# EndMy5uffering/4DGaussianSplatRendering

Hardware: AMD Instinct MI355X
Metric: Gaussians/sec + ms/frame @1080p; sort permutation bit-exact (higher is better)
Workload: dtype f32; 1 GPU; 1,000,000 random 3D splats in a 400^3 cube, single 1080p frame (BASELINE.json configs[1]); splats=1000000, width=1920, height=1080, sort=on, frame_lanes=4, tile_list_entries=1377553, longest_tile_list=477, unordered_draws=3094, staged_list_draws=3094, overflow_reruns=3, depth_sort_passes=3, record_bytes_read_by_projection=64, tiles_composited=14400, tiles=32400, key_index_buffer_pairs=4, lane_streams_rejected_at_create=1

## Files before the change

### 4dgaussiansplatrendering_amd/csrc/gs4d_api.hip

```cpp
#include "gs4d_internal.h"
#include <cstdio>
#include <cstring>
#include <cstdlib>
#include <new>
#include <algorithm>
#include <functional>
#include <vector>
#include <cmath>

using namespace gs4d;

namespace {

constexpr int MAX_LANES = 8;

struct Buffer {
    void* d = nullptr;
    size_t bytes = 0;
    uint64_t version = 0;
    float4* soa = nullptr;
    SoaInfo soa_info;
    size_t soa_n = 0;
    uint64_t soa_version = ~0ull;
    uint64_t soa_builds = 0;
// ... 776 lines not shown
    for (int i = 0; i < 4; ++i) c->u.view[5 * i] = c->u.proj[5 * i] = 1.0f;
    if (const char* ev = getenv("GS4D_LANES")) { const int v = atoi(ev); if (v >= 1 && v <= MAX_LANES) c->nlanes = v; }
    if (const char* ev = getenv("GS4D_FUSE_KEYGEN")) c->defer_order = atoi(ev) != 0;
    if (const char* ev = getenv("GS4D_DRAW_PATH")) { if (!strcmp(ev, "ordered")) c->path_pref = 1; }
    if (const char* ev = getenv("GS4D_RENAME")) c->rename_storage = atoi(ev) != 0;
    if (const char* ev = getenv("GS4D_STAGED_BOX")) c->stage_box_enable = atoi(ev) != 0;
    if (const char* ev = getenv("GS4D_STAGED")) c->stage_enable = atoi(ev) != 0;
    if (const char* ev = getenv("GS4D_SLABS")) { const int v = atoi(ev); if (v >= 1 && v <= (int)V2_MAX_SLABS) { c->slabs = 1; while ((int)c->slabs < v) c->slabs *= 2u; } }
    auto bail = [&](int rc) { g_create_error = c->err; gs4d_destroy(c); return rc; };
    if ((e = create_lane_streams(c)) != hipSuccess) return bail(hipfail(c, e, "hipStreamCreate"));
    for (int i = 0; i < c->nlanes; ++i) {
        Lane& L = c->lanes[i];
        for (hipEvent_t* ev : { &L.ev_emit, &L.ev_tail }) {
            if ((e = hipEventCreateWithFlags(ev, hipEventDisableTiming)) != hipSuccess) return bail(hipfail(c, e, "hipEventCreate"));
            if ((e = hipEventRecord(*ev, L.s)) != hipSuccess) return bail(hipfail(c, e, "hipEventRecord"));
        }
        if ((e = hipHostMalloc((void**)&L.host_total, VERDICT_WORDS * 4, hipHostMallocMapped)) != hipSuccess) return bail(hipfail(c, e, "hipHostMalloc"));
        memset(L.host_total, 0, VERDICT_WORDS * 4);
        if ((e = hipHostGetDevicePointer((void**)&L.host_total_dev, L.host_total, 0)) != hipSuccess) return bail(hipfail(c, e, "hipHostGetDevicePointer"));
        L.depth_sort.err = L.pair_sort.err = L.err_word();
    }
    for (hipEvent_t* ev : { &c->ev_user, &c->ev_readback }) {
        if ((e = hipEventCreateWithFlags(ev, hipEventDisableTiming)) != hipSuccess) return bail(hipfail(c, e, "hipEventCreate"));
    }
    {
        bool ordered = false;
        hipStream_t ls[MAX_LANES];
        for (int i = 0; i < c->nlanes; ++i) ls[i] = c->lanes[i].s;
        if ((e = lds_atomic_order_selftest(ls, c->nlanes, &ordered)) != hipSuccess) return bail(hipfail(c, e, "lds_atomic_order_selftest"));
        c->atomic_rank = ordered;
    }
    const int shape_knob = getenv("GS4D_SORT_SHAPE") ? atoi(getenv("GS4D_SORT_SHAPE")) : 0, rank_knob = getenv("GS4D_SORT_RANK") ? atoi(getenv("GS4D_SORT_RANK")) : 0;
    for (int i = 0; i < c->nlanes; ++i) {
        for (SortScratch* ss : { &c->lanes[i].depth_sort, &c->lanes[i].pair_sort }) { ss->atomic_rank = c->atomic_rank; ss->shape_knob = shape_knob; ss->rank_knob = rank_knob; ss->rb_knob = getenv("GS4D_SORT_RB") ? atoi(getenv("GS4D_SORT_RB")) : 0; }
    }
    int rc = alloc_fbs(c, width, height);
    if (rc) return bail(rc);
    *out = c;
    return GS4D_OK;
}

void gs4d_destroy(gs4d_ctx* c) {
    if (!c) return;
    (void)hipSetDevice(c->device);
    for (int i = 0; i < MAX_LANES; ++i) if (c->lanes[i].s) (void)hipStreamSynchronize(c->lanes[i].s);
    for (auto& b : c->bufs) { if (b.d) (void)hipFree(b.d); if (b.soa) (void)hipFree(b.soa); if (b.bbox_dev) (void)hipFree(b.bbox_dev); if (b.ev_fill) (void)hipEventDestroy(b.ev_fill); if (b.ev_scan) (void)hipEventDestroy(b.ev_scan); }
    for (int i = 0; i < MAX_LANES; ++i) {
        Lane& L = c->lanes[i];
        if (c->fbs[i].mem) (void)hipFree(c->fbs[i].mem);
        if (c->fbs[i].tstate) (void)hipFree(c->fbs[i].tstate);
        if (c->fbs[i].linecnt) (void)hipFree(c->fbs[i].linecnt);
        c->fbs[i].free_planes();
        if (L.line_verts) (void)hipFree(L.line_verts);
        if (L.order_copy) (void)hipFree(L.order_copy);
        if (L.regen_keys) (void)hipFree(L.regen_keys);
        if (L.compact_counts) (void)hipFree(L.compact_counts);
        if (L.spatial_scratch) (void)hipFree(L.spatial_scratch);
        if (L.cut_scratch) (void)hipFree(L.cut_scratch);
        for (auto& sp : L.spare) { if (sp.d) (void)hipFree(sp.d); for (hipEvent_t e : sp.ev) if (e) (void)hipEventDestroy(e); }
        if (L.proj) (void)hipFree(L.proj);
        if (L.trects) (void)hipFree(L.trects);
        if (L.pair_keys) (void)hipFree(L.pair_keys);
        tile_lists_free(L.tl);
        sort_scratch_free(L.depth_sort); sort_scratch_free(L.pair_sort); bin_scratch_free(L.bin);
        if (L.host_total) (void)hipHostFree(L.host_total);
        if (L.ev_emit) (void)hipEventDestroy(L.ev_emit);
        if (L.ev_tail) (void)hipEventDestroy(L.ev_tail);
// ... 920 lines not shown
```

### 4dgaussiansplatrendering_amd/csrc/gs4d_internal.h

```cpp
#pragma once
#include <hip/hip_runtime.h>
#include <stdint.h>
#include <stddef.h>
#include <string>
#include <vector>
#include "../../include/gs4d.h"

namespace gs4d {

constexpr int TILE = 8;
constexpr int PROJ_FLOATS = 16;


enum class Outputs : int { Colour = 0, Aux = 1, Ids = 2 };
constexpr bool has_aux(Outputs o) { return o >= Outputs::Aux; }
constexpr bool has_ids(Outputs o) { return o >= Outputs::Ids; }
static_assert(sizeof(gs4d_record_stat) == 16 && offsetof(gs4d_record_stat, wsum) == 8, "the 64-bit sum is naturally aligned in a 16-byte record");
struct StatOut { gs4d_record_stat* rec = nullptr; uint32_t n = 0; };
struct Target {
    float4* fb; uint32_t* tstate; uint32_t epoch; float4 clear;
    Outputs out; float2* aux; uint32_t* ids;
    const float* z = nullptr;
    StatOut stats;
};

struct Uniforms {
    float view[16];
    float proj[16];
    float time;
    float min_opacity;
};

constexpr int VERDICT_WORDS = 16;
enum TotalWord : int { TOT_ENTRIES = 0, TOT_FLAGS = 1, TOT_COUNT_LO = 2, TOT_COUNT_HI = 3, TOT_LONGEST_LIST = 4, TOT_UNUSED_5 = 5, TOT_UNUSED_6 = 6, TOT_SCAN_ARRIVALS = 7, TOT_TICKET = 8, TOT_ABORT = 9 };
enum HostWord : int { HT_ENTRIES = 0, HT_FLAGS = 1, HT_COUNT_LO = 2, HT_COUNT_HI = 3, HT_ERROR = 4, HT_LONGEST_LIST = 5, HT_LONGEST_RUN = 6, HT_FULLEST_BUCKET = 7, HT_FULLEST_SEG = 8, HT_USED_BOX = 9 };
static_assert(TOT_ABORT < VERDICT_WORDS && HT_USED_BOX < VERDICT_WORDS, "the highest word of either layout fits the arrays");
constexpr uint32_t VF_CAPACITY = 1u, VF_LIST = 2u, VF_STAGED_MISS = 4u;

struct SortScratch {
    uint32_t* keys2 = nullptr; uint32_t* vals2 = nullptr; size_t cap = 0;
    uint32_t* hist = nullptr; size_t hist_cap = 0;
    int flip = 0;
    bool hist_pending = false;
    int acc_flip = 0;
    int hist_bits = 32;
    int hist_rb = 8;
    int rb_knob = 0;
    uint32_t hist_bias = 0;
    uint32_t epoch = 0;
    bool atomic_rank = false;
    int shape_knob = 0, rank_knob = 0;
    uint32_t* totals = nullptr;
    uint32_t* err = nullptr;
    struct Resident { const void* fn = nullptr; uint32_t groups = 0; } resident[16];
};
hipError_t sort_scratch_reserve(hipStream_t st, SortScratch& s, size_t n);
void sort_scratch_free(SortScratch& s);
hipError_t radix_sort_pairs(hipStream_t st, SortScratch& s, uint32_t* keys, uint32_t* vals, size_t n, const uint32_t* n_dev, int key_bits, bool have_hist, bool identity_vals = false);
uint32_t* sort_hist_slot(hipStream_t st, SortScratch& s, size_t n_hint, hipError_t* e_out);
int sort_plan_rb(const SortScratch& s, size_t n, int key_bits);
int sort_plan_passes(int key_bits, int rb);
hipError_t lds_atomic_order_selftest(const hipStream_t* streams, int nstreams, bool* ordered);
enum { SOA_FULL = 0, SOA_SYM = 1, SOA_STATIC3D = 2 };
struct SoaInfo { int layout = SOA_FULL; float consts[8] = { 0 }; };
struct KeySrc;
hipError_t launch_keygen(hipStream_t st, const float4* pos, const float4* sig3, const SoaInfo& info, size_t n, const KeySrc& ks, float* keys, uint32_t* idx, uint32_t* ghist, int rb, uint32_t span, uint32_t* err);

template <class T> inline hipError_t grow_device_array(hipStream_t st, T*& p, size_t& cap, size_t want, size_t elem_bytes = sizeof(T)) {
    if (cap >= want) return hipSuccess;
    hipError_t e = hipStreamSynchronize(st); if (e != hipSuccess) return e;
    if (p) (void)hipFree(p);
    p = nullptr; cap = 0;
    if ((e = hipMalloc(&p, want * elem_bytes)) != hipSuccess) { p = nullptr; return e; }
    cap = want;
    return hipSuccess;
}

constexpr int OS_MAX_PASSES = 4;
constexpr int OS_REPL = 8;
constexpr uint32_t OS_MAX_BINS = 512;
constexpr size_t OS_SLOT_WORDS = (size_t)OS_REPL * OS_MAX_PASSES * OS_MAX_BINS;
#ifdef __HIPCC__
__device__ __forceinline__ void os_hist_clear(uint32_t (*h)[OS_MAX_BINS], uint32_t tid) {
#pragma unroll
// ... 208 lines not shown
```

### 4dgaussiansplatrendering_amd/csrc/sort.hip

```cpp
#include "gs4d_internal.h"
#include <algorithm>
#include <cstdlib>
#include <cstdio>
#include <vector>

namespace gs4d {

__global__ __launch_bounds__(256) void k_keygen(const float4* __restrict__ pos, const float4* __restrict__ sig3, uint32_t n, float t,
                                                float camx, float camy, float camz, float4 vrow2 , int key_mode,
                                                float* __restrict__ keys, uint32_t* __restrict__ idx, uint32_t* __restrict__ ghist , int rb ,
                                                uint32_t bias , uint32_t span , uint32_t* __restrict__ err,
                                                float4 csig3, float cmut ) {
    __shared__ uint32_t h[OS_MAX_PASSES][OS_MAX_BINS];
    os_hist_clear(h, threadIdx.x);
    __syncthreads();
    for (uint32_t i0 = blockIdx.x * 256u; i0 < n; i0 += gridDim.x * 256u) {
        const uint32_t i = i0 + threadIdx.x;
        const bool in = i < n;
        float key = 0.0f;
        if (in) {
            float4 p = pos[i];
            float4 s = csig3;
            if (sig3) s = sig3[i]; else p.w = cmut;
            if (key_mode == GS4D_KEY_REF_INV_EUCLID) {
                float ct = t - p.w;
                float x = p.x + s.x * ct;
                float y = p.y + s.y * ct;
                float z = p.z + s.z * ct;
                float dx = x - camx, dy = y - camy, dz = z - camz;
                key = 1.0f / sqrtf(dx * dx + dy * dy + dz * dz);
            } else {
                float k = (1.0f / s.w) * (t - p.w);
                float x = p.x + k * s.x, y = p.y + k * s.y, z = p.z + k * s.z;
                float zv = ((vrow2.x * x + vrow2.y * y) + vrow2.z * z) + vrow2.w;
                key = 1.0f / fmaxf(-zv, 1e-20f);
            }
// ... 30 lines not shown
struct OsBufs { uint32_t* k[3]; uint32_t* v[3]; };

__device__ __forceinline__ uint32_t wave_incl_scan_u32(uint32_t v, uint32_t lane) {
#pragma unroll
    for (int off = 1; off < 64; off <<= 1) { const uint32_t t = __shfl_up(v, off, 64); if (lane >= (unsigned)off) v += t; }
    return v;
}
__global__ __launch_bounds__(256) void k_os_hist(const uint32_t* __restrict__ keys, uint32_t n_cap, const uint32_t* __restrict__ n_dev, int passes, int rb,
                                                 uint32_t* __restrict__ ghist ) {
    __shared__ uint32_t h[OS_MAX_PASSES][OS_MAX_BINS];
    const uint32_t n = n_dev ? min(*n_dev, n_cap) : n_cap;
    const uint32_t tid = threadIdx.x;
    os_hist_clear(h, tid);
    __syncthreads();
    const uint32_t nvec = n / 4u;
    const uint4* k4 = reinterpret_cast<const uint4*>(keys);
    const uint32_t stride = gridDim.x * 256u;
    for (uint32_t i0 = blockIdx.x * 256u + tid; i0 < nvec; i0 += 4u * stride) {
        uint4 kk[4];
        bool in[4];
#pragma unroll
        for (int u = 0; u < 4; ++u) { const uint32_t i = i0 + u * stride; in[u] = i < nvec; kk[u] = in[u] ? k4[i] : make_uint4(0, 0, 0, 0); }
#pragma unroll
        for (int u = 0; u < 4; ++u) {
            os_hist_add(h, kk[u].x, in[u], passes, rb); os_hist_add(h, kk[u].y, in[u], passes, rb);
            os_hist_add(h, kk[u].z, in[u], passes, rb); os_hist_add(h, kk[u].w, in[u], passes, rb);
        }
    }
    if (blockIdx.x == 0) { const bool in = tid < (n & 3u); os_hist_add(h, in ? keys[nvec * 4u + tid] : 0u, in, passes, rb); }
    __syncthreads();
    os_hist_flush(h, ghist, passes, tid);
}

__device__ __forceinline__ bool os_schedule(uint32_t live, int passes, int p, int& src, int& dst, int& executed, int& total) {
    const uint32_t all = (1u << passes) - 1u;
    live &= all;
    int k = __popc(live);
    if (k == 1) { const uint32_t deadm = all & ~live; live |= deadm & (0u - deadm); ++k; }
    total = k;
    const int j = __popc(live & ((1u << p) - 1u));
    executed = j;
    if (!((live >> p) & 1u)) return false;
    auto buf_at = [k](int i) { if (k & 1) { if (i <= 2) return i; return (i - 3) & 1; } return i & 1; };
    src = buf_at(j);
    dst = buf_at(j + 1);
    return true;
}

__device__ __forceinline__ uint32_t os_tword(uint32_t epoch, uint32_t count) { return ((epoch & 0x3FFFFu) << 14) | count; }
__device__ __forceinline__ bool os_tpublished(uint32_t w, uint32_t epoch) { return (w >> 14) == (epoch & 0x3FFFFu); }


template <int LB, int BINS>
__device__ __forceinline__ uint32_t os_tiles_finish(const uint32_t* st, int32_t hi, int rows, int k0, uint32_t sum, uint32_t tid, uint32_t epoch, uint32_t* err) {
    uint32_t spins = 0;
    while (true) {
        while (true) {
            __builtin_amdgcn_s_sleep(8);
            const uint32_t w = __hip_atomic_load(st + (size_t)(hi - k0) * (uint32_t)BINS + tid, __ATOMIC_RELAXED, __HIP_MEMORY_SCOPE_AGENT);
            if (os_tpublished(w, epoch)) { sum += w & 0x3FFFu; break; }
            if (++spins > (1u << 20)) { __hip_atomic_store(err, 1u, __ATOMIC_RELAXED, __HIP_MEMORY_SCOPE_SYSTEM); return sum; }
        }
        if (++k0 >= rows) return sum;
        uint32_t sv[LB];
#pragma unroll
        for (int k = 0; k < LB; ++k) sv[k] = (k >= k0 && k < rows) ? __hip_atomic_load(st + (size_t)(hi - k) * (uint32_t)BINS + tid, __ATOMIC_RELAXED, __HIP_MEMORY_SCOPE_AGENT) : 0u;
        bool missing = false;
#pragma unroll
        for (int k = 0; k < LB; ++k) {
            if (missing || k < k0 || k >= rows) continue;
            if (!os_tpublished(sv[k], epoch)) { k0 = k; missing = true; continue; }
            sum += sv[k] & 0x3FFFu;
        }
        if (!missing) return sum;
    }
}

template <int LB, int BINS>
__device__ __forceinline__ uint32_t os_acc_finish(const uint32_t* acc, uint32_t t, int rows, int k0, uint32_t sum, uint32_t expect, uint32_t tid, uint32_t* err) {
// ... 48 lines not shown
    const uint32_t* sacc = acc + (size_t)acc_groups * (uint32_t)BINS;
    for (uint32_t t = 0; t < sup; t += 16u) {
        const int rows = (int)min(16u, sup - t);
        uint32_t sv[16];
#pragma unroll
        for (int k = 0; k < 16; ++k) sv[k] = k < rows ? __hip_atomic_load(sacc + (size_t)(t + k) * (uint32_t)BINS + tid, __ATOMIC_RELAXED, __HIP_MEMORY_SCOPE_AGENT) : 0u;
        int miss = -1;
#pragma unroll
        for (int k = 0; k < 16; ++k) {
            if (miss >= 0 || k >= rows) continue;
            if ((sv[k] >> 24) != OS_SUPER) { miss = k; continue; }
            sum_s += sv[k] & 0xFFFFFFu;
        }
        if (miss >= 0) sum_s = os_acc_finish<16, BINS>(sacc, t, rows, miss, sum_s, OS_SUPER, tid, err);
    }
    if (miss_t >= 0) sum_t = os_tiles_finish<(int)OS_GROUP, BINS>(st, hi, rows_t, miss_t, sum_t, tid, epoch, err);
    if (miss_g >= 0) sum_g = os_acc_finish<(int)OS_SUPER, BINS>(acc, g0, rows_g, miss_g, sum_g, OS_GROUP, tid, err);
    return sum_t + sum_g + sum_s;
}

template <int THREADS, int BINS>
__device__ __forceinline__ uint32_t digit_excl_scan(uint32_t v, uint32_t* tmp , uint32_t tid) {
    const uint32_t lane = tid & 63u, w = tid >> 6;
    const uint32_t inc = wave_incl_scan_u32(tid < (uint32_t)BINS ? v : 0u, lane);
    __syncthreads();
    if (lane == 63u && w < (uint32_t)(BINS / 64)) tmp[w] = inc;
    __syncthreads();
    uint32_t base = 0;
#pragma unroll
    for (int k = 0; k < BINS / 64 - 1; ++k) if ((unsigned)k < w) base += tmp[k];
    return base + inc - v;
}

template <int THREADS, int ITEMS, bool ATOMIC_RANK, int RB>
__global__ __launch_bounds__(THREADS) void k_os_pass(OsBufs bufs, uint32_t n_cap, const uint32_t* __restrict__ n_dev, int pass, int passes,
                                                     const uint32_t* __restrict__ ghist , uint32_t* __restrict__ ghist_other ,
                                                     uint32_t* status , uint32_t* acc , uint32_t* acc_next , uint32_t acc_groups, uint32_t acc_words,
                                                     uint32_t epoch, uint32_t* err,
                                                     uint32_t* ticket , uint32_t* ticket_next , uint32_t bias, int identity_vals ,
                                                     u64* stamps ) {
    constexpr uint32_t TILE_KEYS = THREADS * ITEMS;
    constexpr int WAVES = THREADS / 64;
    constexpr uint32_t BINS = 1u << RB;
    static_assert(BINS <= (uint32_t)THREADS && BINS <= OS_MAX_BINS && BINS >= 64u, "one thread per digit");
    static_assert(TILE_KEYS < (1u << 14), "tile-level look-back words carry 14-bit counts");
    static_assert((uint64_t)TILE_KEYS * OS_GROUP * OS_SUPER < (1u << 24) && OS_GROUP < 256u && OS_SUPER < 256u, "accumulators are {arrivals:8, sum:24}");
    __shared__ uint32_t skeys[TILE_KEYS];
    __shared__ uint32_t svals[TILE_KEYS];
    __shared__ uint32_t wcnt[WAVES][BINS];
    __shared__ uint32_t loff[BINS];
    __shared__ uint32_t gpos[BINS];
    __shared__ uint32_t s_tmp[BINS / 64];
    __shared__ uint32_t s_dead;
    __shared__ uint32_t s_tile;

    const uint32_t n = n_dev ? min(*n_dev, n_cap) : n_cap;
    const uint32_t tid = threadIdx.x, lane = tid & 63u, w = tid >> 6;
    if (tid == 0) s_tile = atomicAdd(ticket, 1u);
    if (tid == 1u) s_dead = 0u;
    if (tid == 2u && blockIdx.x == 0) __hip_atomic_store(ticket_next, 0u, __ATOMIC_RELAXED, __HIP_MEMORY_SCOPE_AGENT);
    for (uint32_t q = tid; q < WAVES * BINS; q += THREADS) (&wcnt[0][0])[q] = 0u;
    uint32_t tot = 0, dead = 0;
    if (tid < BINS) {
        for (int q = 0; q < passes; ++q) {
            uint32_t g = 0;
#pragma unroll
            for (int r = 0; r < OS_REPL; ++r) g += ghist[(r * OS_MAX_PASSES + q) * OS_MAX_BINS + tid];
            if (q == pass) tot = g;
            if (g == n) dead |= 1u << q;
        }
    }
    __syncthreads();
    if (dead) atomicOr(&s_dead, dead);
    const uint32_t ntiles = (n + TILE_KEYS - 1u) / TILE_KEYS;
    for (uint32_t q = blockIdx.x * THREADS + tid; q < acc_words; q += gridDim.x * THREADS) acc_next[q] = 0u;
    if (pass == 0 && blockIdx.x == 0) { for (uint32_t q = tid; q < OS_SLOT_WORDS; q += THREADS) ghist_other[q] = 0u; }
    __syncthreads();
    uint32_t tile = s_tile;
    if (tile >= ntiles) return;
    const int shift = RB * pass;
    int src, dst, executed, total;
    if (!os_schedule(~s_dead, passes, pass, src, dst, executed, total)) {
        if (identity_vals && pass == 0 && total == 0) { for (uint32_t i = blockIdx.x * THREADS + tid; i < n; i += gridDim.x * THREADS) bufs.v[0][i] = i; }
        return;
    }
    const bool make_identity = identity_vals && executed == 0;
    const uint32_t* __restrict__ keys_in = bufs.k[src]; const uint32_t* __restrict__ vals_in = bufs.v[src];
    uint32_t* __restrict__ keys_out = bufs.k[dst]; uint32_t* __restrict__ vals_out = bufs.v[dst];
    uint32_t digit_base = 0;
    bool first = true;
    const uint32_t ngroups = (ntiles + OS_GROUP - 1u) / OS_GROUP, nsuper = (ngroups + OS_SUPER - 1u) / OS_SUPER;

    while (true) {
        OS_STAMP(0);
        const uint32_t tbase = tile * TILE_KEYS;
        const uint32_t wbase = tbase + w * (64u * ITEMS);
        uint32_t key[ITEMS], val[ITEMS], rank[ITEMS];
#pragma unroll
        for (int j = 0; j < ITEMS; ++j) {
            const uint32_t i = wbase + j * 64u + lane;
            const bool valid = i < n;
            key[j] = valid ? keys_in[i] : 0xFFFFFFFFu;
            val[j] = !valid ? 0u : make_identity ? i : vals_in[i];
        }
        if (first) { digit_base = digit_excl_scan<THREADS, (int)BINS>(tot, s_tmp, tid); first = false; }
        OS_STAMP(1);

        if (ATOMIC_RANK) {
#pragma unroll
            for (int j = 0; j < ITEMS; ++j) {
                const bool valid = (wbase + j * 64u + lane) < n;
                const uint32_t d = ((key[j] - bias) >> shift) & (BINS - 1u);
                rank[j] = valid ? atomicAdd(&wcnt[w][d], 1u) : 0u;
            }
        } else {
            const uint64_t lt = (1ull << lane) - 1ull;
            volatile uint32_t* wc = wcnt[w];
#pragma unroll
            for (int j = 0; j < ITEMS; ++j) {
                const bool valid = (wbase + j * 64u + lane) < n;
                const uint32_t d = ((key[j] - bias) >> shift) & (BINS - 1u);
                uint64_t m = __ballot(valid);
#pragma unroll
                for (int b = 0; b < RB; ++b) {
                    const bool bit = (d >> b) & 1u;
                    const uint64_t bal = __ballot(bit);
                    m &= bit ? bal : ~bal;
                }
                rank[j] = 0;
                if (valid) {
                    const uint32_t c = wc[d];
                    rank[j] = c + (uint32_t)__popcll(m & lt);
                    __builtin_amdgcn_wave_barrier();
                    if ((m & lt) == 0) wc[d] = c + (uint32_t)__popcll(m);
                }
                __builtin_amdgcn_wave_barrier();
            }
        }
        __syncthreads();
        uint32_t cnt = 0;
        uint32_t garr = 0;
        const uint32_t grp = tile / OS_GROUP, sup = grp / OS_SUPER;
        if (tid < BINS) {
#pragma unroll
            for (int k = 0; k < WAVES; ++k) { const uint32_t t = wcnt[k][tid]; wcnt[k][tid] = cnt; cnt += t; }
            __hip_atomic_store(status + (size_t)tile * BINS + tid, os_tword(epoch, cnt), __ATOMIC_RELAXED, __HIP_MEMORY_SCOPE_AGENT);
            if (sup + 1u < nsuper) garr = __hip_atomic_fetch_add(acc + (size_t)grp * BINS + tid, (1u << 24) | cnt, __ATOMIC_RELAXED, __HIP_MEMORY_SCOPE_AGENT);
            else if (grp + 1u < ngroups) (void)__hip_atomic_fetch_add(acc + (size_t)grp * BINS + tid, (1u << 24) | cnt, __ATOMIC_RELAXED, __HIP_MEMORY_SCOPE_AGENT);
        }
        OS_STAMP(2);
        const uint32_t lo_ = digit_excl_scan<THREADS, (int)BINS>(cnt, s_tmp, tid);
        if (tid < BINS) loff[tid] = lo_;
        __syncthreads();
#pragma unroll
        for (int j = 0; j < ITEMS; ++j) {
            if ((wbase + j * 64u + lane) < n) {
                const uint32_t d = ((key[j] - bias) >> shift) & (BINS - 1u);
                const uint32_t l = loff[d] + wcnt[w][d] + rank[j];
                skeys[l] = key[j];
                svals[l] = val[j];
            }
        }
        OS_STAMP(3);
        if (tid < BINS) {
            if (sup + 1u < nsuper && (garr >> 24) == OS_GROUP - 1u)
                (void)__hip_atomic_fetch_add(acc + (size_t)(acc_groups + sup) * BINS + tid, (1u << 24) | ((garr & 0xFFFFFFu) + cnt), __ATOMIC_RELAXED, __HIP_MEMORY_SCOPE_AGENT);
            const uint32_t prefix = os_lookback<(int)BINS>(status, acc, acc_groups, tile, tid, epoch, err);
            gpos[tid] = digit_base + prefix;
        }
        __syncthreads();
        OS_STAMP(4);
        const uint32_t tcount = min(TILE_KEYS, n - tbase);
#pragma unroll
        for (int j = 0; j < ITEMS; ++j) {
            const uint32_t l = j * THREADS + tid;
            if (l < tcount) {
                const uint32_t k = skeys[l];
                const uint32_t d = ((k - bias) >> shift) & (BINS - 1u);
                const uint32_t o = gpos[d] + (l - loff[d]);
                if (o >= n) { __hip_atomic_store(err, 3u, __ATOMIC_RELAXED, __HIP_MEMORY_SCOPE_SYSTEM); continue; }
                if (ITEMS >= 12) { keys_out[o] = k; vals_out[o] = svals[l]; }
                else { __builtin_nontemporal_store(k, keys_out + o); __builtin_nontemporal_store(svals[l], vals_out + o); }
            }
        }
        OS_STAMP(5);
        if (gridDim.x >= ntiles) return;
        uint32_t next = 0;
        if (tid == 0) next = atomicAdd(ticket, 1u);
        __syncthreads();
        if (tid == 0) s_tile = next;
        for (uint32_t q = tid; q < WAVES * BINS; q += THREADS) (&wcnt[0][0])[q] = 0u;
        __syncthreads();
        tile = s_tile;
        if (tile >= ntiles) return;
    }
}

__global__ __launch_bounds__(256) void k_lds_order_test(uint32_t* __restrict__ bad) {
    __shared__ uint32_t cnt[4][256];
    const uint32_t tid = threadIdx.x, lane = tid & 63u, w = tid >> 6;
    uint32_t errors = 0;
    for (uint32_t round = 0; round < 96u; ++round) {
#pragma unroll
        for (int k = 0; k < 4; ++k) cnt[k][tid] = 0u;
        __syncthreads();
        const uint32_t bins = round % 6u == 0u ? 1u : round % 6u == 1u ? 2u : round % 6u == 2u ? 3u : round % 6u == 3u ? 7u : round % 6u == 4u ? 64u : 256u;
        uint32_t x = (blockIdx.x * 256u + tid) * 2654435761u + round * 40503u; x ^= x >> 15; x *= 2246822519u; x ^= x >> 13;
        const uint32_t d = x % bins;
        const bool active = ((x >> 20) & 7u) != 0u;
        uint64_t m = __ballot(active);
#pragma unroll
        for (int b = 0; b < 8; ++b) { const bool bit = (d >> b) & 1u; const uint64_t bal = __ballot(bit); m &= bit ? bal : ~bal; }
        if (active) {
            const uint32_t got = atomicAdd(&cnt[w][d], 1u);
            const uint32_t want = (uint32_t)__popcll(m & ((1ull << lane) - 1ull));
            if (got != want) ++errors;
            const uint32_t got2 = atomicAdd(&cnt[w][d], 1u);
            if (got2 != (uint32_t)__popcll(m) + want) ++errors;
        }
        __syncthreads();
    }
    if (errors) atomicAdd(bad, errors);
}

hipError_t lds_atomic_order_selftest(const hipStream_t* streams, int nstreams, bool* ordered) {
    *ordered = false;
    if (nstreams < 1) return hipErrorInvalidValue;
    if (nstreams > 8) nstreams = 8;
    uint32_t* d = nullptr; uint32_t h[8] = { 1, 1, 1, 1, 1, 1, 1, 1 };
    hipError_t e = hipMalloc(&d, 4 * (size_t)nstreams);
    if (e != hipSuccess) return e;
    for (int i = 0; i < nstreams && e == hipSuccess; ++i) e = hipMemsetAsync(d + i, 0, 4, streams[i]);
    for (int i = 0; i < nstreams && e == hipSuccess; ++i) { k_lds_order_test<<<dim3(512), dim3(256), 0, streams[i]>>>(d + i); e = hipGetLastError(); }
    for (int i = 0; i < nstreams && e == hipSuccess; ++i) e = hipMemcpyAsync(&h[i], d + i, 4, hipMemcpyDeviceToHost, streams[i]);
    for (int i = 0; i < nstreams; ++i) { const hipError_t e2 = hipStreamSynchronize(streams[i]); if (e == hipSuccess) e = e2; }
    (void)hipFree(d);
    bool ok = e == hipSuccess;
    for (int i = 0; i < nstreams; ++i) ok = ok && h[i] == 0;
    *ordered = ok;
    return e;
}

hipError_t sort_scratch_reserve(hipStream_t st, SortScratch& s, size_t n) {
    hipError_t e;
    if (s.cap < n) {
        e = grow_device_array(st, s.keys2, s.cap, n, 16);
        s.vals2 = s.keys2 ? s.keys2 + 2 * s.cap : nullptr;
        if (e != hipSuccess) return e;
    }
    const size_t tiles = (s.cap + 1023) / 1024;
    const size_t groups = tiles / OS_GROUP + 2, supers = groups / OS_SUPER + 2;
    const size_t words = 2 * OS_SLOT_WORDS + (tiles + 2 + 2 * 2 * (groups + supers)) * OS_MAX_BINS;
    if (s.hist_cap < words) {
        uint32_t* nh = nullptr;
        if ((e = hipMalloc(&nh, words * 4)) != hipSuccess) return e;
        if ((e = hipMemsetAsync(nh, 0, words * 4, st)) != hipSuccess) return e;
        if (s.hist) {
            if ((e = hipMemcpyAsync(nh, s.hist, 2 * OS_SLOT_WORDS * 4, hipMemcpyDeviceToDevice, st)) != hipSuccess) return e;
            (void)hipStreamSynchronize(st); (void)hipFree(s.hist);
        }
        s.hist = nh; s.hist_cap = words;
    }
    if (!s.totals) {
        if (const char* e0 = getenv("GS4D_TEST_EPOCH0")) s.epoch = (uint32_t)strtoul(e0, nullptr, 0);
    }
    if (!s.totals) { if ((e = hipMalloc(&s.totals, 256 * 4)) != hipSuccess) return e; if ((e = hipMemsetAsync(s.totals, 0, 1024, st)) != hipSuccess) return e; }
    return hipSuccess;
}

void sort_scratch_free(SortScratch& s) {
    if (s.keys2) (void)hipFree(s.keys2);
    if (s.hist) (void)hipFree(s.hist);
    if (s.totals) (void)hipFree(s.totals);
    s = SortScratch();
}

uint32_t* sort_hist_slot(hipStream_t st, SortScratch& s, size_t n_hint, hipError_t* e_out) {
    hipError_t e = sort_scratch_reserve(st, s, n_hint);
    if (e == hipSuccess && s.hist_pending) e = hipMemsetAsync(s.hist + (s.flip ? OS_SLOT_WORDS : 0), 0, OS_SLOT_WORDS * 4, st);
    if (e_out) *e_out = e;
    if (e != hipSuccess) return nullptr;
    s.hist_pending = true;
    return s.hist + (s.flip ? OS_SLOT_WORDS : 0);
}

template <int THREADS, int ITEMS, bool ATOMIC_RANK, int RB>
static hipError_t onesweep(hipStream_t st, SortScratch& s, uint32_t* keys, uint32_t* vals, size_t n, const uint32_t* n_dev, int passes, bool have_hist, bool identity_vals) {
    const uint32_t tile_keys = THREADS * ITEMS;
    const uint32_t tiles = (uint32_t)((n + tile_keys - 1) / tile_keys);
    uint32_t resident = 0;
    {
        const void* const fn = reinterpret_cast<const void*>(&k_os_pass<THREADS, ITEMS, ATOMIC_RANK, RB>);
        SortScratch::Resident* slot = nullptr;
        for (auto& r : s.resident) { if (r.fn == fn) { resident = r.groups; break; } if (!r.fn && !slot) slot = &r; }
        if (!resident) {
            int per_cu = 0, dev = 0, cus = 0;
            if (hipOccupancyMaxActiveBlocksPerMultiprocessor(&per_cu, k_os_pass<THREADS, ITEMS, ATOMIC_RANK, RB>, THREADS, 0) != hipSuccess || per_cu < 1) per_cu = 1;
            if (hipGetDevice(&dev) != hipSuccess || hipDeviceGetAttribute(&cus, hipDeviceAttributeMultiprocessorCount, dev) != hipSuccess || cus < 1) cus = 256;
            resident = (uint32_t)per_cu * (uint32_t)cus;
            if (slot) { slot->fn = fn; slot->groups = resident; }
        }
    }
    const uint32_t grid = std::min(tiles, resident);
    uint32_t* ghist = s.hist + (s.flip ? OS_SLOT_WORDS : 0);
    uint32_t* ghist_other = s.hist + (s.flip ? 0 : OS_SLOT_WORDS);
    hipError_t e;
    const uint32_t bias = have_hist ? s.hist_bias : 0u;
    s.hist_bias = 0;
    if (!have_hist) {
        if (s.hist_pending) { if ((e = hipMemsetAsync(ghist, 0, OS_SLOT_WORDS * 4, st)) != hipSuccess) return e; }
        const uint32_t hist_blocks = (uint32_t)std::min<size_t>((n / 16 + 255) / 256 + 1, 256);
        k_os_hist<<<dim3(hist_blocks), dim3(256), 0, st>>>(keys, (uint32_t)n, n_dev, passes, RB, ghist);
    }
    s.hist_pending = false;
    s.flip ^= 1;
#ifdef GS4D_TUNING
    static const char* stampf = getenv("GS4D_SORT_STAMP_FILE");
    static const int stamp_pass = getenv("GS4D_SORT_STAMP_PASS") ? atoi(getenv("GS4D_SORT_STAMP_PASS")) : 0;
#else
    const char* stampf = nullptr; const int stamp_pass = 0;
#endif
    u64* stamps = nullptr;
    if (stampf && hipMalloc(&stamps, (size_t)tiles * 64) != hipSuccess) stamps = nullptr;
    uint32_t* status = s.hist + 2 * OS_SLOT_WORDS;
    const size_t cap_tiles = (s.cap + 1023) / 1024, cap_groups = cap_tiles / OS_GROUP + 2, cap_supers = cap_groups / OS_SUPER + 2;
    const size_t acc_words = (cap_groups + cap_supers) * OS_MAX_BINS;
    uint32_t* acc_base = status + (cap_tiles + 2) * OS_MAX_BINS;
    OsBufs b;
    b.k[0] = keys; b.v[0] = vals;
    b.k[1] = s.keys2; b.v[1] = s.vals2;
    b.k[2] = s.keys2 + s.cap; b.v[2] = s.vals2 + s.cap;
    for (int p = 0; p < passes; ++p) {
        ++s.epoch;
        if ((s.epoch & 0x3FFFFu) == 0u) {
            if ((e = hipMemsetAsync(status, 0, (s.hist_cap - 2 * OS_SLOT_WORDS) * 4, st)) != hipSuccess) return e;
            ++s.epoch;
        }
        k_os_pass<THREADS, ITEMS, ATOMIC_RANK, RB><<<dim3(grid), dim3(THREADS), 0, st>>>(b, (uint32_t)n, n_dev, p, passes, ghist, ghist_other, status, acc_base + (s.acc_flip ? acc_words : 0), acc_base + (s.acc_flip ? 0 : acc_words), (uint32_t)cap_groups, (uint32_t)acc_words,
                                                                         s.epoch & 0x3FFFFFFFu,
                                                                         s.err ? s.err : s.totals, s.totals + 64 + (s.acc_flip ? 1 : 0), s.totals + 64 + (s.acc_flip ? 0 : 1), bias, identity_vals ? 1 : 0, (stampf && p == stamp_pass) ? stamps : nullptr);
        s.acc_flip ^= 1;
    }
    if (stampf && stamps) {
        (void)hipStreamSynchronize(st);
        std::vector<u64> hs((size_t)tiles * 8);
        (void)hipMemcpy(hs.data(), stamps, hs.size() * 8, hipMemcpyDeviceToHost);
        FILE* f = fopen(stampf, "w");
        if (f) { for (uint32_t t = 0; t < tiles; ++t) { for (int k = 0; k < 6; ++k) fprintf(f, "%llu ", hs[t * 8 + k] - hs[0]); fprintf(f, "\n"); } fclose(f); }
        (void)hipFree(stamps);
    }
    return hipGetLastError();
}

int sort_plan_rb(const SortScratch& s, size_t n, int key_bits) {
    (void)n;
    if (s.rb_knob == 8 || s.rb_knob == 9) return (s.rb_knob == 9 && (s.shape_knob == 1 || s.shape_knob == 4)) ? 8 : s.rb_knob;
    if (s.shape_knob == 1 || s.shape_knob == 4) return 8;
    const int p8 = std::max(2, (key_bits + 7) / 8), p9 = std::max(2, (key_bits + 8) / 9);
    return p9 < p8 ? 9 : 8;
}
int sort_plan_passes(int key_bits, int rb) { return std::min(OS_MAX_PASSES, std::max(2, (key_bits + rb - 1) / rb)); }

hipError_t radix_sort_pairs(hipStream_t st, SortScratch& s, uint32_t* keys, uint32_t* vals, size_t n, const uint32_t* n_dev, int key_bits, bool have_hist, bool identity_vals) {
    if (n <= 1) { if (n == 1 && identity_vals) return hipMemsetAsync(vals, 0, 4, st); return hipSuccess; }
    if (n >= (1ull << 32) - 1) return hipErrorInvalidValue;
    hipError_t e = sort_scratch_reserve(st, s, n);
    if (e != hipSuccess) return e;
    const int rb = have_hist ? s.hist_rb : sort_plan_rb(s, n, key_bits);
    if (rb != 8 && rb != 9) return hipErrorInvalidValue;
    const int passes = sort_plan_passes(key_bits, rb);
    int shape = s.shape_knob ? s.shape_knob : 5;
    (void)n;
    if (rb == 9 && shape == 5 && !s.shape_knob) shape = 6;
// ... 18 lines not shown
```

Before: 10.61 billion splats/s.

## Add opt-in single-launch onesweep radix sort with cross-pass done counters

Adds a variant of the onesweep pass kernel that runs all digit passes in one launch. Work items are ordered pass-major and blocks spin on per-pass done counters before starting the next pass, replacing separate kernel launches with in-kernel dependency waits and a second alternating accumulator buffer. It is gated behind GS4D_SORT_ONE_LAUNCH and defaults off. The change also adds a grid-size knob and a min-waves launch bound for 512-thread configurations, which can change register allocation on the default path.

```diff
diff --git a/4dgaussiansplatrendering_amd/csrc/gs4d_api.hip b/4dgaussiansplatrendering_amd/csrc/gs4d_api.hip
--- a/4dgaussiansplatrendering_amd/csrc/gs4d_api.hip
+++ b/4dgaussiansplatrendering_amd/csrc/gs4d_api.hip
@@ -832,7 +832,8 @@
     }
     const int shape_knob = getenv("GS4D_SORT_SHAPE") ? atoi(getenv("GS4D_SORT_SHAPE")) : 0, rank_knob = getenv("GS4D_SORT_RANK") ? atoi(getenv("GS4D_SORT_RANK")) : 0;
     for (int i = 0; i < c->nlanes; ++i) {
-        for (SortScratch* ss : { &c->lanes[i].depth_sort, &c->lanes[i].pair_sort }) { ss->atomic_rank = c->atomic_rank; ss->shape_knob = shape_knob; ss->rank_knob = rank_knob; ss->rb_knob = getenv("GS4D_SORT_RB") ? atoi(getenv("GS4D_SORT_RB")) : 0; }
+        for (SortScratch* ss : { &c->lanes[i].depth_sort, &c->lanes[i].pair_sort }) { ss->atomic_rank = c->atomic_rank; ss->shape_knob = shape_knob; ss->rank_knob = rank_knob; ss->rb_knob = getenv("GS4D_SORT_RB") ? atoi(getenv("GS4D_SORT_RB")) : 0;
+                                                                                   ss->one_launch_knob = getenv("GS4D_SORT_ONE_LAUNCH") ? (atoi(getenv("GS4D_SORT_ONE_LAUNCH")) != 0) : -1; ss->grid_knob = getenv("GS4D_SORT_GRID") ? atoi(getenv("GS4D_SORT_GRID")) : 0; }
     }
     int rc = alloc_fbs(c, width, height);
     if (rc) return bail(rc);
diff --git a/4dgaussiansplatrendering_amd/csrc/gs4d_internal.h b/4dgaussiansplatrendering_amd/csrc/gs4d_internal.h
--- a/4dgaussiansplatrendering_amd/csrc/gs4d_internal.h
+++ b/4dgaussiansplatrendering_amd/csrc/gs4d_internal.h
@@ -50,6 +50,9 @@
     uint32_t epoch = 0;
     bool atomic_rank = false;
     int shape_knob = 0, rank_knob = 0;
+    int one_launch_knob = -1;
+    int grid_knob = 0;
+    int done_flip = 0;
     uint32_t* totals = nullptr;
     uint32_t* err = nullptr;
     struct Resident { const void* fn = nullptr; uint32_t groups = 0; } resident[16];
diff --git a/4dgaussiansplatrendering_amd/csrc/sort.hip b/4dgaussiansplatrendering_amd/csrc/sort.hip
--- a/4dgaussiansplatrendering_amd/csrc/sort.hip
+++ b/4dgaussiansplatrendering_amd/csrc/sort.hip
@@ -2,6 +2,7 @@
 #include <algorithm>
 #include <cstdlib>
 #include <cstdio>
+#include <type_traits>
 #include <vector>
 
 namespace gs4d {
@@ -98,11 +99,15 @@
     os_hist_flush(h, ghist, passes, tid);
 }
 
-__device__ __forceinline__ bool os_schedule(uint32_t live, int passes, int p, int& src, int& dst, int& executed, int& total) {
+__device__ __forceinline__ uint32_t os_executed_mask(uint32_t live, int passes) {
     const uint32_t all = (1u << passes) - 1u;
     live &= all;
-    int k = __popc(live);
-    if (k == 1) { const uint32_t deadm = all & ~live; live |= deadm & (0u - deadm); ++k; }
+    if (__popc(live) == 1) { const uint32_t deadm = all & ~live; live |= deadm & (0u - deadm); }
+    return live;
+}
+__device__ __forceinline__ bool os_schedule(uint32_t live, int passes, int p, int& src, int& dst, int& executed, int& total) {
+    live = os_executed_mask(live, passes);
+    const int k = __popc(live);
     total = k;
     const int j = __popc(live & ((1u << p) - 1u));
     executed = j;
@@ -111,6 +116,10 @@
     src = buf_at(j);
     dst = buf_at(j + 1);
     return true;
+}
+__device__ __forceinline__ int os_nth_executed(uint32_t executed_mask, int j) {
+    for (int k = 0; k < j; ++k) executed_mask &= executed_mask - 1u;
+    return __ffs((int)executed_mask) - 1;
 }
 
 __device__ __forceinline__ uint32_t os_tword(uint32_t epoch, uint32_t count) { return ((epoch & 0x3FFFFu) << 14) | count; }
@@ -225,16 +234,19 @@
     return base + inc - v;
 }
 
-template <int THREADS, int ITEMS, bool ATOMIC_RANK, int RB>
-__global__ __launch_bounds__(THREADS) void k_os_pass(OsBufs bufs, uint32_t n_cap, const uint32_t* __restrict__ n_dev, int pass, int passes,
+#define OS_MIN_WAVES(T, I, R) (((T) == 512 && !((I) == 16 && (R) == 9)) ? 4 : 1)
+template <int THREADS, int ITEMS, bool ATOMIC_RANK, int RB, bool ONE>
+__global__ __launch_bounds__(THREADS, OS_MIN_WAVES(THREADS, ITEMS, RB)) void k_os_pass(OsBufs bufs, uint32_t n_cap, const uint32_t* __restrict__ n_dev, int pass , int passes,
                                                      const uint32_t* __restrict__ ghist , uint32_t* __restrict__ ghist_other ,
                                                      uint32_t* status , uint32_t* acc , uint32_t* acc_next , uint32_t acc_groups, uint32_t acc_words,
                                                      uint32_t epoch, uint32_t* err,
                                                      uint32_t* ticket , uint32_t* ticket_next , uint32_t bias, int identity_vals ,
-                                                     u64* stamps ) {
+                                                     u64* stamps ,
+                                                     uint32_t* acc_mid , uint32_t* done , uint32_t* done_next ) {
     constexpr uint32_t TILE_KEYS = THREADS * ITEMS;
     constexpr int WAVES = THREADS / 64;
     constexpr uint32_t BINS = 1u << RB;
+    constexpr uint32_t OS_ABANDON = 0xFFFFFFFFu;
     static_assert(BINS <= (uint32_t)THREADS && BINS <= OS_MAX_BINS && BINS >= 64u, "one thread per digit");
     static_assert(TILE_KEYS < (1u << 14), "tile-level look-back words carry 14-bit counts");
     static_assert((uint64_t)TILE_KEYS * OS_GROUP * OS_SUPER < (1u << 24) && OS_GROUP < 256u && OS_SUPER < 256u, "accumulators are {arrivals:8, sum:24}");
@@ -252,37 +264,93 @@
     if (tid == 0) s_tile = atomicAdd(ticket, 1u);
     if (tid == 1u) s_dead = 0u;
     if (tid == 2u && blockIdx.x == 0) __hip_atomic_store(ticket_next, 0u, __ATOMIC_RELAXED, __HIP_MEMORY_SCOPE_AGENT);
+    if (ONE && tid >= 64u && tid < 64u + (uint32_t)OS_MAX_PASSES && blockIdx.x == 0) __hip_atomic_store(done_next + (tid - 64u), 0u, __ATOMIC_RELAXED, __HIP_MEMORY_SCOPE_AGENT);
     for (uint32_t q = tid; q < WAVES * BINS; q += THREADS) (&wcnt[0][0])[q] = 0u;
     uint32_t tot = 0, dead = 0;
+    uint32_t totq[OS_MAX_PASSES] = { 0u, 0u, 0u, 0u };
+    static_assert(OS_MAX_PASSES == 4, "totq");
     if (tid < BINS) {
-        for (int q = 0; q < passes; ++q) {
-            uint32_t g = 0;
-#pragma unroll
-            for (int r = 0; r < OS_REPL; ++r) g += ghist[(r * OS_MAX_PASSES + q) * OS_MAX_BINS + tid];
-            if (q == pass) tot = g;
-            if (g == n) dead |= 1u << q;
+        if (ONE) {
+#pragma unroll
+            for (int q = 0; q < OS_MAX_PASSES; ++q) {
+                if (q >= passes) continue;
+                uint32_t g = 0;
+#pragma unroll
+                for (int r = 0; r < OS_REPL; ++r) g += ghist[(r * OS_MAX_PASSES + q) * OS_MAX_BINS + tid];
+                totq[q] = g;
+                if (g == n) dead |= 1u << q;
+            }
+        } else {
+            for (int q = 0; q < passes; ++q) {
+                uint32_t g = 0;
+#pragma unroll
+                for (int r = 0; r < OS_REPL; ++r) g += ghist[(r * OS_MAX_PASSES + q) * OS_MAX_BINS + tid];
+                if (q == pass) tot = g;
+                if (g == n) dead |= 1u << q;
+            }
         }
     }
     __syncthreads();
     if (dead) atomicOr(&s_dead, dead);
     const uint32_t ntiles = (n + TILE_KEYS - 1u) / TILE_KEYS;
     for (uint32_t q = blockIdx.x * THREADS + tid; q < acc_words; q += gridDim.x * THREADS) acc_next[q] = 0u;
-    if (pass == 0 && blockIdx.x == 0) { for (uint32_t q = tid; q < OS_SLOT_WORDS; q += THREADS) ghist_other[q] = 0u; }
+    if ((ONE || pass == 0) && blockIdx.x == 0) { for (uint32_t q = tid; q < OS_SLOT_WORDS; q += THREADS) ghist_other[q] = 0u; }
     __syncthreads();
     uint32_t tile = s_tile;
-    if (tile >= ntiles) return;
-    const int shift = RB * pass;
-    int src, dst, executed, total;
-    if (!os_schedule(~s_dead, passes, pass, src, dst, executed, total)) {
-        if (identity_vals && pass == 0 && total == 0) { for (uint32_t i = blockIdx.x * THREADS + tid; i < n; i += gridDim.x * THREADS) bufs.v[0][i] = i; }
-        return;
-    }
-    const bool make_identity = identity_vals && executed == 0;
-    const uint32_t* __restrict__ keys_in = bufs.k[src]; const uint32_t* __restrict__ vals_in = bufs.v[src];
-    uint32_t* __restrict__ keys_out = bufs.k[dst]; uint32_t* __restrict__ vals_out = bufs.v[dst];
+    uint32_t item = tile, nitems = ntiles;
+    int shift = RB * pass;
+    int src = 0, dst = 0, executed = 0, total = 0;
+    int cur_j = 0;
+    uint32_t ep = epoch;
+    uint32_t* acc_cur = acc;
+    bool first = true;
+    if (ONE) {
+        const uint32_t xm = os_executed_mask(~s_dead, passes);
+        total = __popc(xm);
+        if (total == 0) {
+            if (identity_vals) { for (uint32_t i = blockIdx.x * THREADS + tid; i < n; i += gridDim.x * THREADS) bufs.v[0][i] = i; }
+            return;
+        }
+        nitems = ntiles * (uint32_t)total;
+        if (item >= nitems) return;
+        cur_j = (int)(item / ntiles);
+        tile = item - (uint32_t)cur_j * ntiles;
+        if (cur_j > 0) {
+            if (tid == 0) {
+                uint32_t spins = 0;
+                while (__hip_atomic_load(done + (cur_j - 1), __ATOMIC_RELAXED, __HIP_MEMORY_SCOPE_AGENT) < ntiles) {
+                    __builtin_amdgcn_s_sleep(8);
+                    if (++spins > (1u << 20)) { __hip_atomic_store(err, 1u, __ATOMIC_RELAXED, __HIP_MEMORY_SCOPE_SYSTEM); s_tile = OS_ABANDON; break; }
+                }
+                __builtin_amdgcn_fence(__ATOMIC_ACQUIRE, "agent");
+                asm volatile("s_waitcnt vmcnt(0)" ::: "memory");
+            }
+            __syncthreads();
+            if (s_tile == OS_ABANDON) return;
+        }
+        const int p = os_nth_executed(xm, cur_j);
+        (void)os_schedule(~s_dead, passes, p, src, dst, executed, total);
+        shift = RB * p;
+        tot = p == 0 ? totq[0] : p == 1 ? totq[1] : p == 2 ? totq[2] : totq[3];
+        ep = epoch + (uint32_t)cur_j;
+        acc_cur = (cur_j & 1) ? acc_mid : acc;
+    } else {
+        if (tile >= ntiles) return;
+        if (!os_schedule(~s_dead, passes, pass, src, dst, executed, total)) {
+            if (identity_vals && pass == 0 && total == 0) { for (uint32_t i = blockIdx.x * THREADS + tid; i < n; i += gridDim.x * THREADS) bufs.v[0][i] = i; }
+            return;
+        }
+    }
+    bool make_identity = identity_vals && executed == 0;
+    using In = std::conditional_t<ONE, const uint32_t*, const uint32_t* __restrict__>;
+    using Out = std::conditional_t<ONE, uint32_t*, uint32_t* __restrict__>;
+    In keys_in = bufs.k[src]; In vals_in = bufs.v[src];
+    Out keys_out = bufs.k[dst]; Out vals_out = bufs.v[dst];
     uint32_t digit_base = 0;
-    bool first = true;
     const uint32_t ngroups = (ntiles + OS_GROUP - 1u) / OS_GROUP, nsuper = (ngroups + OS_SUPER - 1u) / OS_SUPER;
+#ifdef GS4D_TUNING
+    if (ONE && stamps && shift != RB * pass) stamps = nullptr;
+#endif
 
     while (true) {
         OS_STAMP(0);
@@ -337,9 +405,15 @@
         if (tid < BINS) {
 #pragma unroll
             for (int k = 0; k < WAVES; ++k) { const uint32_t t = wcnt[k][tid]; wcnt[k][tid] = cnt; cnt += t; }
-            __hip_atomic_store(status + (size_t)tile * BINS + tid, os_tword(epoch, cnt), __ATOMIC_RELAXED, __HIP_MEMORY_SCOPE_AGENT);
-            if (sup + 1u < nsuper) garr = __hip_atomic_fetch_add(acc + (size_t)grp * BINS + tid, (1u << 24) | cnt, __ATOMIC_RELAXED, __HIP_MEMORY_SCOPE_AGENT);
-            else if (grp + 1u < ngroups) (void)__hip_atomic_fetch_add(acc + (size_t)grp * BINS + tid, (1u << 24) | cnt, __ATOMIC_RELAXED, __HIP_MEMORY_SCOPE_AGENT);
+            __hip_atomic_store(status + (size_t)tile * BINS + tid, os_tword(ep, cnt), __ATOMIC_RELAXED, __HIP_MEMORY_SCOPE_AGENT);
+            if (sup + 1u < nsuper) garr = __hip_atomic_fetch_add(acc_cur + (size_t)grp * BINS + tid, (1u << 24) | cnt, __ATOMIC_RELAXED, __HIP_MEMORY_SCOPE_AGENT);
+            else if (grp + 1u < ngroups) (void)__hip_atomic_fetch_add(acc_cur + (size_t)grp * BINS + tid, (1u << 24) | cnt, __ATOMIC_RELAXED, __HIP_MEMORY_SCOPE_AGENT);
+        }
+        if (ONE && cur_j + 1 < total) {
+            uint32_t* const z = (cur_j & 1) ? acc : acc_mid;
+            const uint32_t zg = ngroups * BINS, zw = zg + nsuper * BINS, per = (zw + ntiles - 1u) / ntiles;
+            for (uint32_t q = tile * per + tid; q < min(zw, (tile + 1u) * per); q += THREADS)
+                __hip_atomic_store(z + (q < zg ? (size_t)q : (size_t)acc_groups * BINS + (q - zg)), 0u, __ATOMIC_RELAXED, __HIP_MEMORY_SCOPE_AGENT);
         }
         OS_STAMP(2);
         const uint32_t lo_ = digit_excl_scan<THREADS, (int)BINS>(cnt, s_tmp, tid);
@@ -357,8 +431,8 @@
         OS_STAMP(3);
         if (tid < BINS) {
             if (sup + 1u < nsuper && (garr >> 24) == OS_GROUP - 1u)
-                (void)__hip_atomic_fetch_add(acc + (size_t)(acc_groups + sup) * BINS + tid, (1u << 24) | ((garr & 0xFFFFFFu) + cnt), __ATOMIC_RELAXED, __HIP_MEMORY_SCOPE_AGENT);
-            const uint32_t prefix = os_lookback<(int)BINS>(status, acc, acc_groups, tile, tid, epoch, err);
+                (void)__hip_atomic_fetch_add(acc_cur + (size_t)(acc_groups + sup) * BINS + tid, (1u << 24) | ((garr & 0xFFFFFFu) + cnt), __ATOMIC_RELAXED, __HIP_MEMORY_SCOPE_AGENT);
+            const uint32_t prefix = os_lookback<(int)BINS>(status, acc_cur, acc_groups, tile, tid, ep, err);
             gpos[tid] = digit_base + prefix;
         }
         __syncthreads();
@@ -377,15 +451,66 @@
             }
         }
         OS_STAMP(5);
-        if (gridDim.x >= ntiles) return;
-        uint32_t next = 0;
-        if (tid == 0) next = atomicAdd(ticket, 1u);
-        __syncthreads();
-        if (tid == 0) s_tile = next;
-        for (uint32_t q = tid; q < WAVES * BINS; q += THREADS) (&wcnt[0][0])[q] = 0u;
-        __syncthreads();
-        tile = s_tile;
-        if (tile >= ntiles) return;
+        if (!ONE) {
+            if (gridDim.x >= ntiles) return;
+            uint32_t next = 0;
+            if (tid == 0) next = atomicAdd(ticket, 1u);
+            __syncthreads();
+            if (tid == 0) s_tile = next;
+            for (uint32_t q = tid; q < WAVES * BINS; q += THREADS) (&wcnt[0][0])[q] = 0u;
+            __syncthreads();
+            tile = s_tile;
+            if (tile >= ntiles) return;
+        } else {
+            const bool boundary = cur_j + 1 < total;
+            const bool early = gridDim.x >= ntiles;
+            uint32_t next = 0;
+            if (early && tid == 0) next = atomicAdd(ticket, 1u);
+            if (boundary) asm volatile("s_waitcnt vmcnt(0)" ::: "memory");
+            __syncthreads();
+            if (tid == 0) {
+                if (boundary) {
+                    __builtin_amdgcn_fence(__ATOMIC_RELEASE, "agent");
+                    asm volatile("s_waitcnt vmcnt(0)" ::: "memory");
+                    (void)__hip_atomic_fetch_add(done + cur_j, 1u, __ATOMIC_RELAXED, __HIP_MEMORY_SCOPE_AGENT);
+                }
+                if (!early) next = atomicAdd(ticket, 1u);
+                const int nj = next < nitems ? (int)(next / ntiles) : cur_j;
+                if (nj != cur_j) {
+                    uint32_t spins = 0;
+                    while (__hip_atomic_load(done + (nj - 1), __ATOMIC_RELAXED, __HIP_MEMORY_SCOPE_AGENT) < ntiles) {
+                        __builtin_amdgcn_s_sleep(8);
+                        if (++spins > (1u << 20)) { __hip_atomic_store(err, 1u, __ATOMIC_RELAXED, __HIP_MEMORY_SCOPE_SYSTEM); next = OS_ABANDON; break; }
+                    }
+                    __builtin_amdgcn_fence(__ATOMIC_ACQUIRE, "agent");
+                    asm volatile("s_waitcnt vmcnt(0)" ::: "memory");
+                }
+                s_tile = next;
+            }
+            for (uint32_t q = tid; q < WAVES * BINS; q += THREADS) (&wcnt[0][0])[q] = 0u;
+            __syncthreads();
+            item = s_tile;
+            if (item >= nitems) return;
+            const int nj = (int)(item / ntiles);
+            tile = item - (uint32_t)nj * ntiles;
+            if (nj != cur_j) {
+                cur_j = nj;
+                const uint32_t xm = os_executed_mask(~s_dead, passes);
+                const int p = os_nth_executed(xm, cur_j);
+                (void)os_schedule(~s_dead, passes, p, src, dst, executed, total);
+                shift = RB * p;
+                tot = p == 0 ? totq[0] : p == 1 ? totq[1] : p == 2 ? totq[2] : totq[3];
+                first = true;
+                ep = epoch + (uint32_t)cur_j;
+                acc_cur = (cur_j & 1) ? acc_mid : acc;
+                make_identity = false;
+                keys_in = bufs.k[src]; vals_in = bufs.v[src];
+                keys_out = bufs.k[dst]; vals_out = bufs.v[dst];
+#ifdef GS4D_TUNING
+                stamps = nullptr;
+#endif
+            }
+        }
     }
 }
 
@@ -443,7 +568,7 @@
     }
     const size_t tiles = (s.cap + 1023) / 1024;
     const size_t groups = tiles / OS_GROUP + 2, supers = groups / OS_SUPER + 2;
-    const size_t words = 2 * OS_SLOT_WORDS + (tiles + 2 + 2 * 2 * (groups + supers)) * OS_MAX_BINS;
+    const size_t words = 2 * OS_SLOT_WORDS + (tiles + 2 + 4 * (groups + supers)) * OS_MAX_BINS;
     if (s.hist_cap < words) {
         uint32_t* nh = nullptr;
         if ((e = hipMalloc(&nh, words * 4)) != hipSuccess) return e;
@@ -477,24 +602,28 @@
     return s.hist + (s.flip ? OS_SLOT_WORDS : 0);
 }
 
+template <class K>
+static uint32_t os_resident(SortScratch& s, K kernel, int threads) {
+    const void* const fn = reinterpret_cast<const void*>(kernel);
+    SortScratch::Resident* slot = nullptr;
+    for (auto& r : s.resident) { if (r.fn == fn) return r.groups; if (!r.fn && !slot) slot = &r; }
+    int per_cu = 0, dev = 0, cus = 0;
+    if (hipOccupancyMaxActiveBlocksPerMultiprocessor(&per_cu, kernel, threads, 0) != hipSuccess || per_cu < 1) per_cu = 1;
+    if (hipGetDevice(&dev) != hipSuccess || hipDeviceGetAttribute(&cus, hipDeviceAttributeMultiprocessorCount, dev) != hipSuccess || cus < 1) cus = 256;
+    const uint32_t resident = (uint32_t)per_cu * (uint32_t)cus;
+    if (slot) { slot->fn = fn; slot->groups = resident; }
+    return resident;
+}
+
 template <int THREADS, int ITEMS, bool ATOMIC_RANK, int RB>
 static hipError_t onesweep(hipStream_t st, SortScratch& s, uint32_t* keys, uint32_t* vals, size_t n, const uint32_t* n_dev, int passes, bool have_hist, bool identity_vals) {
     const uint32_t tile_keys = THREADS * ITEMS;
     const uint32_t tiles = (uint32_t)((n + tile_keys - 1) / tile_keys);
     uint32_t resident = 0;
-    {
-        const void* const fn = reinterpret_cast<const void*>(&k_os_pass<THREADS, ITEMS, ATOMIC_RANK, RB>);
-        SortScratch::Resident* slot = nullptr;
-        for (auto& r : s.resident) { if (r.fn == fn) { resident = r.groups; break; } if (!r.fn && !slot) slot = &r; }
-        if (!resident) {
-            int per_cu = 0, dev = 0, cus = 0;
-            if (hipOccupancyMaxActiveBlocksPerMultiprocessor(&per_cu, k_os_pass<THREADS, ITEMS, ATOMIC_RANK, RB>, THREADS, 0) != hipSuccess || per_cu < 1) per_cu = 1;
-            if (hipGetDevice(&dev) != hipSuccess || hipDeviceGetAttribute(&cus, hipDeviceAttributeMultiprocessorCount, dev) != hipSuccess || cus < 1) cus = 256;
-            resident = (uint32_t)per_cu * (uint32_t)cus;
-            if (slot) { slot->fn = fn; slot->groups = resident; }
-        }
-    }
-    const uint32_t grid = std::min(tiles, resident);
+    const bool one = s.one_launch_knob == 1;
+    if (one) resident = os_resident(s, &k_os_pass<THREADS, ITEMS, ATOMIC_RANK, RB, true>, THREADS);
+    if (!one) resident = os_resident(s, &k_os_pass<THREADS, ITEMS, ATOMIC_RANK, RB, false>, THREADS);
+    const uint32_t grid = std::min(std::min(tiles, resident), s.grid_knob > 0 ? (uint32_t)s.grid_knob : 0xFFFFFFFFu);
     uint32_t* ghist = s.hist + (s.flip ? OS_SLOT_WORDS : 0);
     uint32_t* ghist_other = s.hist + (s.flip ? 0 : OS_SLOT_WORDS);
     hipError_t e;
@@ -523,15 +652,32 @@
     b.k[0] = keys; b.v[0] = vals;
     b.k[1] = s.keys2; b.v[1] = s.vals2;
     b.k[2] = s.keys2 + s.cap; b.v[2] = s.vals2 + s.cap;
-    for (int p = 0; p < passes; ++p) {
+    uint32_t* const errw = s.err ? s.err : s.totals;
+    if (one) {
+        if (((s.epoch + 1u) & 0x3FFFFu) == 0u || ((s.epoch + 1u) & 0x3FFFFu) + (uint32_t)passes - 1u > 0x3FFFFu) {
+            if ((e = hipMemsetAsync(status, 0, (s.hist_cap - 2 * OS_SLOT_WORDS) * 4, st)) != hipSuccess) return e;
+            s.epoch |= 0x3FFFFu;
+            ++s.epoch;
+        }
+        const uint32_t epoch0 = s.epoch + 1u;
+        s.epoch += (uint32_t)passes;
+        k_os_pass<THREADS, ITEMS, ATOMIC_RANK, RB, true><<<dim3(grid), dim3(THREADS), 0, st>>>(b, (uint32_t)n, n_dev, stamp_pass, passes, ghist, ghist_other, status, acc_base + (s.acc_flip ? acc_words : 0), acc_base + (s.acc_flip ? 0 : acc_words), (uint32_t)cap_groups, (uint32_t)acc_words,
+                                                                         epoch0 & 0x3FFFFFFFu,
+                                                                         errw, s.totals + 64 + (s.acc_flip ? 1 : 0), s.totals + 64 + (s.acc_flip ? 0 : 1), bias, identity_vals ? 1 : 0, stampf ? stamps : nullptr,
+                                                                         acc_base + 2 * acc_words, s.totals + 72 + (s.done_flip ? OS_MAX_PASSES : 0), s.totals + 72 + (s.done_flip ? 0 : OS_MAX_PASSES));
+        s.acc_flip ^= 1;
+        s.done_flip ^= 1;
+    }
+    for (int p = 0; p < passes && !one; ++p) {
         ++s.epoch;
         if ((s.epoch & 0x3FFFFu) == 0u) {
             if ((e = hipMemsetAsync(status, 0, (s.hist_cap - 2 * OS_SLOT_WORDS) * 4, st)) != hipSuccess) return e;
             ++s.epoch;
         }
-        k_os_pass<THREADS, ITEMS, ATOMIC_RANK, RB><<<dim3(grid), dim3(THREADS), 0, st>>>(b, (uint32_t)n, n_dev, p, passes, ghist, ghist_other, status, acc_base + (s.acc_flip ? acc_words : 0), acc_base + (s.acc_flip ? 0 : acc_words), (uint32_t)cap_groups, (uint32_t)acc_words,
+        k_os_pass<THREADS, ITEMS, ATOMIC_RANK, RB, false><<<dim3(grid), dim3(THREADS), 0, st>>>(b, (uint32_t)n, n_dev, p, passes, ghist, ghist_other, status, acc_base + (s.acc_flip ? acc_words : 0), acc_base + (s.acc_flip ? 0 : acc_words), (uint32_t)cap_groups, (uint32_t)acc_words,
                                                                          s.epoch & 0x3FFFFFFFu,
-                                                                         s.err ? s.err : s.totals, s.totals + 64 + (s.acc_flip ? 1 : 0), s.totals + 64 + (s.acc_flip ? 0 : 1), bias, identity_vals ? 1 : 0, (stampf && p == stamp_pass) ? stamps : nullptr);
+                                                                         errw, s.totals + 64 + (s.acc_flip ? 1 : 0), s.totals + 64 + (s.acc_flip ? 0 : 1), bias, identity_vals ? 1 : 0, (stampf && p == stamp_pass) ? stamps : nullptr,
+                                                                         nullptr, nullptr, nullptr);
         s.acc_flip ^= 1;
     }
     if (stampf && stamps) {
```

Result: slower. 10.18 billion splats/s (-4.0%).
